# mikelodder7/bls-bn254

Hardware: AMD Instinct MI355X
Metric: BN254 pairings/sec (= BLS verifies/sec) (higher is better)
Workload: dtype int64; 1 GPU; 262144 batched single-sig BLS verifies per GPU (BASELINE configs[1]), unique 32-byte messages, 1024-key pool, 1/64 invalid tuples; key de-duplication + hash-to-G1 + per-key G2 checks and line tables + 2-pair Miller loop + final exp; tuples_per_gpu=262144, tuples_total=262144, key_pool=1024

## Files before the change

bls-bn254_amd/csrc/curve.h:

```cpp
#pragma once
#include "tower.h"

namespace bn {

BN_INL Fp f_add(const Fp& a, const Fp& b) { return fp_add(a, b); }
BN_INL Fp f_sub(const Fp& a, const Fp& b) { return fp_sub(a, b); }
BN_INL Fp f_mul(const Fp& a, const Fp& b) { return fp_mul(a, b); }
BN_INL Fp f_sqr(const Fp& a) { return fp_sqr(a); }
BN_INL Fp f_norm(const Fp& a) { return fp_norm(a); }
BN_INL Fp f_neg(const Fp& a) { return fp_neg(a); }
BN_INL bool f_is_zero(const Fp& a) { return fp_is_zero(a); }
BN_INL Fp f_select(bool c, const Fp& a, const Fp& b) { return fp_select(c, a, b); }
BN_INL Fp f_mul_b3(const Fp& a) { return fp_lc2<9, 0>(a, a); }
template <int K1, int K2> BN_INL Fp f_lc2(const Fp& a, const Fp& b) { return fp_lc2<K1, K2>(a, b); }
template <int K1, int K2, int K3> BN_INL Fp f_lc3(const Fp& a, const Fp& b, const Fp& c) { return fp_lc3<K1, K2, K3>(a, b, c); }
BN_INL void f_set_zero(Fp& a) { a = fp_zero(); }
BN_INL void f_set_one(Fp& a) { a = fp_one(); }

BN_INL Fp2 f_add(const Fp2& a, const Fp2& b) { return fp2_add(a, b); }
BN_INL Fp2 f_sub(const Fp2& a, const Fp2& b) { return fp2_sub(a, b); }
BN_INL Fp2 f_mul(const Fp2& a, const Fp2& b) { return fp2_mul(a, b); }
BN_INL Fp2 f_sqr(const Fp2& a) { return fp2_sqr(a); }
BN_INL Fp2 f_norm(const Fp2& a) { return fp2_norm(a); }
BN_INL Fp2 f_neg(const Fp2& a) { return fp2_neg(a); }
// ... 60 lines not shown
template <class F> BN_FUNC Proj<F> proj_dbl(const Proj<F>& a) {
  BN_CTX;
  F t0 = f_sqr(a.y);
  F z8 = f_lc2<8, 0>(t0, t0);
  F t1 = f_mul(a.y, a.z);
  F t2 = f_mul_b3(f_sqr(a.z));
  F x3 = f_mul(t2, z8);
  F y3 = f_norm(f_add(t0, t2));
  F z3 = f_mul(t1, z8);
  F t0m = f_lc2<1, -3>(t0, t2);
  F yy = f_norm(f_add(x3, f_mul(t0m, y3)));
  F xy = f_mul(a.x, a.y);
  F xx = f_lc2<2, 0>(f_mul(t0m, xy), t0);
  return {xx, yy, z3};
}
template <class F> BN_FUNC Proj<F> jac_dbl(const Proj<F>& p) {
  BN_CTX;
  F A = f_sqr(p.x), B = f_sqr(p.y);
  F C = f_sqr(B);
  F t = f_sqr(f_norm(f_add(p.x, B)));
  F D = f_lc3<2, -2, -2>(t, A, C);
  F E = f_lc2<3, 0>(A, A);
  F x3 = f_lc2<1, -2>(f_sqr(E), D);
  F y3 = f_lc2<1, -8>(f_mul(E, f_norm(f_sub(D, x3))), C);
  F yz = f_mul(p.y, p.z);
  return {x3, y3, f_lc2<2, 0>(yz, yz)};
}
template <class F> BN_FUNC Proj<F> proj_to_jac(const Proj<F>& p) {
  BN_CTX;
  return {f_mul(p.x, p.z), f_mul(p.y, f_sqr(p.z)), p.z};
}
template <class F> BN_FUNC Proj<F> proj_from_jac(const Proj<F>& j) {
  BN_CTX;
  bool inf = f_is_zero(j.z);
  Proj<F> id = proj_identity<F>();
  Proj<F> r = {f_mul(j.x, j.z), j.y, f_mul(f_sqr(j.z), j.z)};
  return {f_select(inf, id.x, r.x), f_select(inf, id.y, r.y), f_select(inf, id.z, r.z)};
}
template <class F> BN_INL Proj<F> proj_neg(const Proj<F>& a) { return {a.x, f_norm(f_neg(a.y)), a.z}; }
template <class F> BN_INL Proj<F> proj_select(bool c, const Proj<F>& a, const Proj<F>& b) {
  return {f_select(c, a.x, b.x), f_select(c, a.y, b.y), f_select(c, a.z, b.z)};
}
template <class F> BN_FUNC Proj<F> proj_mul_u64(const Proj<F>& p, uint64_t k) {
  BN_CTX;
  Proj<F> acc = proj_identity<F>();
  for (int i = 63; i >= 0; --i) {
    acc = proj_dbl(acc);
    if ((k >> i) & 1) acc = proj_add(acc, p);
  }
  return acc;
}
struct ChainOp { int8_t load, sq, mul, store, cstore; };
constexpr int BN_X_CHAIN_LEN = 13, BN_X_CHAIN_SLOTS = 5;
#define BN_X_CHAIN {{-1, 4, 0, 1, 2}, {-1, 1, 0, 3, 4}, {-1, 6, 4, -1, -1}, {-1, 7, 1, -1, -1}, {-1, 2, 3, -1, -1}, {-1, 4, 4, -1, -1}, {-1, 4, 4, -1, -1}, \
                    {-1, 9, 3, -1, -1}, {-1, 4, 3, -1, -1}, {-1, 6, 1, -1, -1}, {-1, 5, 3, -1, -1}, {-1, 5, 2, -1, -1}, {-1, 5, 1, -1, -1}}
template <class F> BN_FUNC Proj<F> proj_mul_bn_x(const Proj<F>& p) {
  BN_CTX;
  const ChainOp prog[BN_X_CHAIN_LEN] = BN_X_CHAIN;
  Proj<F> slot[BN_X_CHAIN_SLOTS];
  slot[0] = p;
  Proj<F> r = p;
  for (int k = 0; k < BN_X_CHAIN_LEN; ++k) {
    const ChainOp op = prog[k];
    if (op.load >= 0) r = slot[op.load];
    if (op.sq >= 2) {
      Proj<F> j = proj_to_jac(r);
      for (int q = 0; q < op.sq; ++q) j = jac_dbl(j);
      r = proj_from_jac(j);
    } else if (op.sq == 1) r = proj_dbl(r);
    if (op.mul >= 0) r = proj_add(r, slot[op.mul]);
    if (op.store >= 0) slot[op.store] = r;
    if (op.cstore >= 0) slot[op.cstore] = proj_neg(r);
  }
  return r;
}
template <class F> BN_FUNC Proj<F> proj_mul_256(const Proj<F>& p, const uint64_t* k) {
  BN_CTX;
  Proj<F> acc = proj_identity<F>();
  for (int i = 255; i >= 0; --i) {
    acc = proj_dbl(acc);
    Proj<F> s = proj_add(acc, p);
    acc = proj_select((k[i >> 6] >> (i & 63)) & 1, s, acc);
  }
  return acc;
}
template <class F> BN_FUNC Proj<F> proj_mul_win4(const Proj<F>& p, const uint64_t* k) {
  BN_CTX;
  Proj<F> tab[16];
  tab[0] = proj_identity<F>();
  tab[1] = p;
  for (int i = 2; i < 16; ++i) tab[i] = proj_add(tab[i - 1], p);
  Proj<F> acc = tab[(int)(k[3] >> 60)];
  for (int w = 62; w >= 0; --w) {
    const int d = (int)((k[w >> 4] >> ((w & 15) * 4)) & 15);
    const Proj<F> t = tab[d];
    acc = proj_dbl(proj_dbl(proj_dbl(proj_dbl(acc))));
    acc = proj_add(acc, t);
  }
  return acc;
}
template <class F> BN_INL bool proj_eq(const Proj<F>& a, const Proj<F>& b) {
  bool ai = f_is_zero(a.z), bi = f_is_zero(b.z);
  bool e = f_is_zero(f_sub(f_mul(a.x, b.z), f_mul(b.x, a.z))) & f_is_zero(f_sub(f_mul(a.y, b.z), f_mul(b.y, a.z)));
  return (ai | bi) ? (ai & bi) : e;
}

BN_INL G1A g1_decode(const uint8_t* b, bool& ok) {
  bool okx, oky;
// ... 102 lines not shown
}
BN_FUNC G1A svdw_g1_finish(const Fp& u_in, const Fp& tv3) {
  BN_CTX;
  Fp u = fp_norm(u_in);
  Fp c2 = fp_const(bnc::SVDW1_C2), c3 = fp_const(bnc::SVDW1_C3), c4 = fp_const(bnc::SVDW1_C4), one = fp_one(), b = fp_const(bnc::THREE);
  Fp u2 = fp_sqr(u);
  Fp tv1 = fp_lc2<4, 0>(u2, u2);
  Fp tv2 = fp_norm(fp_add(one, tv1));
  tv1 = fp_norm(fp_sub(one, tv1));
  Fp tv4 = fp_mul(fp_mul(fp_mul(u, tv1), tv3), c3);
  Fp x1 = fp_norm(fp_sub(c2, tv4));
  Fp gx1 = fp_norm(fp_add(fp_mul(fp_sqr(x1), x1), b));
  Fp x2 = fp_norm(fp_add(c2, tv4));
  Fp gx2 = fp_norm(fp_add(fp_mul(fp_sqr(x2), x2), b));
  Fp x3 = fp_mul(fp_sqr(tv2), tv3);
  x3 = fp_norm(fp_add(fp_mul(fp_sqr(x3), c4), one));
  Fp gx3 = fp_norm(fp_add(fp_mul(fp_sqr(x3), x3), b));
  bool e1 = fp_is_square(gx1), e2 = fp_is_square(gx2), sq;
  G1A r;
  r.x = fp_select(e1, x1, fp_select(e2, x2, x3));
  Fp y = fp_sqrt_cand(fp_select(e1, gx1, fp_select(e2, gx2, gx3)), sq);
  bool flip = fp_sgn0(u) != fp_sgn0(y);
  r.y = fp_select(flip, fp_norm(fp_neg(y)), y);
  r.inf = false;
  return r;
}
BN_FUNC G1A svdw_g1(const Fp& u) { return svdw_g1_finish(u, fp_inv(svdw_g1_den(u))); }
struct SvdwFrac { Fp n, d, y; };
BN_FUNC SvdwFrac svdw_g1_frac(const Fp& u_in) {
  BN_CTX;
  const Fp u = fp_norm(u_in);
  const Fp c2 = fp_const(bnc::SVDW1_C2), c3 = fp_const(bnc::SVDW1_C3), c4 = fp_const(bnc::SVDW1_C4), one = fp_one();
  const Fp u2 = fp_sqr(u);
  Fp tv1 = fp_lc2<4, 0>(u2, u2);
  const Fp tv2 = fp_norm(fp_add(one, tv1));
  tv1 = fp_norm(fp_sub(one, tv1));
  const bool exc = fp_is_zero(tv1) | fp_is_zero(tv2);
  const Fp c3u = fp_mul(c3, u), c2t = fp_mul(c2, tv2);
  const Fp n1 = fp_select(exc, c2, fp_norm(fp_sub(c2t, c3u))), n2 = fp_select(exc, c2, fp_norm(fp_add(c2t, c3u)));
  const Fp d12 = fp_select(exc, one, tv2);
  const Fp t1s = fp_sqr(tv1);
  const Fp d3 = fp_select(exc, one, fp_norm(t1s));
  const Fp n3 = fp_select(exc, one, fp_norm(fp_add(t1s, fp_mul(c4, fp_sqr(tv2)))));
  const Fp v12 = fp_mul(fp_sqr(d12), d12), v3 = fp_mul(fp_sqr(d3), d3);
  const Fp g1n = fp_norm(fp_add(fp_mul(fp_sqr(n1), n1), fp_lc2<3, 0>(v12, v12)));
  const Fp g2n = fp_norm(fp_add(fp_mul(fp_sqr(n2), n2), fp_lc2<3, 0>(v12, v12)));
  const Fp g3n = fp_norm(fp_add(fp_mul(fp_sqr(n3), n3), fp_lc2<3, 0>(v3, v3)));
  const bool e1 = fp_is_square(fp_mul(g1n, d12)), e2 = fp_is_square(fp_mul(g2n, d12));
  SvdwFrac r;
  r.n = fp_select(e1, n1, fp_select(e2, n2, n3));
  r.d = fp_select(e1 | e2, d12, d3);
  const Fp U = fp_select(e1, g1n, fp_select(e2, g2n, g3n)), V = fp_select(e1 | e2, v12, v3);
  const Fp V3 = fp_mul(fp_sqr(V), V);
  const Fp y = fp_mul(fp_mul(U, V), fp_pow(fp_mul(U, V3), BN_EXP(EXP_PM3_4)));
  const bool flip = fp_sgn0(u) != fp_sgn0(y);
  r.y = fp_select(flip, fp_norm(fp_neg(y)), y);
  return r;
}
BN_FUNC G1P hash_to_g1_from_fields_proj(const Fp& u0, const Fp& u1) {
  BN_CTX;
#if defined(__HIP_DEVICE_COMPILE__) && defined(BN_HASH_MAP_LOOP)
  Fp u[2] = {u0, u1};
  G1P q[2];
  _Pragma("unroll 1") for (int k = 0; k < 2; ++k) {
    const SvdwFrac a = svdw_g1_frac(u[k]);
    q[k] = G1P{a.n, fp_mul(a.y, a.d), a.d};
  }
  return proj_add(q[0], q[1]);
#else
  const SvdwFrac a = svdw_g1_frac(u0), b = svdw_g1_frac(u1);
  const G1P q0 = {a.n, fp_mul(a.y, a.d), a.d}, q1 = {b.n, fp_mul(b.y, b.d), b.d};
  return proj_add(q0, q1);
#endif
}
BN_FUNC G1A hash_to_g1_from_fields(const Fp& u0, const Fp& u1) { return g1_to_affine(hash_to_g1_from_fields_proj(u0, u1)); }

BN_FUNC Fp2 fp2_pow(const Fp2& a, Exp256 e) {
  BN_CTX;
  Fp2 base = fp2_norm(a), r = fp2_one();
  for (int i = 255; i >= 0; --i) {
    r = fp2_sqr(r);
    Fp2 m = fp2_mul(r, base);
    r = fp2_select((e.w[i >> 6] >> (i & 63)) & 1, m, r);
  }
  return r;
}
BN_FUNC bool fp2_is_square(const Fp2& a) {
  Fp2 n = fp2_norm(a);
  return fp_is_square(fp_dot2(n.c0, n.c0, n.c1, n.c1));
}
BN_FUNC Fp2 fp2_sqrt(const Fp2& a_in) {
  BN_CTX;
  Fp2 a = fp2_norm(a_in);
  Fp2 a1 = fp2_pow(a, BN_EXP(EXP_PM3_4));
  Fp2 alpha = fp2_mul(fp2_sqr(a1), a);
  Fp2 x0 = fp2_mul(a1, a);
  bool neg_one = fp2_is_zero(fp2_add(alpha, fp2_one()));
  Fp2 alt = {fp_norm(fp_neg(x0.c1)), x0.c0};
  Fp2 b = fp2_pow(fp2_norm(fp2_add(alpha, fp2_one())), BN_EXP(EXP_PM1_2));
  Fp2 r = fp2_mul(b, x0);
  return fp2_select(neg_one, alt, r);
}
BN_FUNC G2A g2_decompress(const uint8_t* in, bool& ok) {
  uint8_t xb[32];
  for (int i = 0; i < 32; ++i) xb[i] = in[i];
  int flag = xb[0] >> 7; xb[0] &= 0x7f;
  bool o0, o1;
// ... 39 lines not shown
```

bls-bn254_amd/csrc/fp29.h:

```cpp
#pragma once
#include <stdint.h>
#include "bn254_consts.h"

#if defined(__HIPCC__)
#include <hip/hip_runtime.h>
#define BN_HD __host__ __device__
#else
#define BN_HD
#endif
#define BN_INL BN_HD inline __attribute__((always_inline))
#ifdef BN_FORCE_INLINE
#define BN_FUNC BN_INL
#else
#define BN_FUNC BN_HD inline
#endif

#define BN_UNROLL _Pragma("unroll")
#if defined(__HIP_DEVICE_COMPILE__)
#define BN_SCHED_BARRIER __builtin_amdgcn_sched_barrier(0)
#else
#define BN_SCHED_BARRIER ((void)0)
#endif

#ifdef BN_CHECK
#include <cmath>
#include <cstdio>
#include <cstdlib>
#endif

namespace bn {

constexpr int NL = 9;
constexpr int RB = 29;
constexpr int32_t MASK = (1 << RB) - 1;

struct Fp {
  int32_t l[NL];
#ifdef BN_CHECK
  double lo = 0, hi = 0;
  double tlo = 0, thi = 0;
  double vb = 0;
#endif
};

#ifdef BN_CHECK
struct CheckStats { double worst_mul = 0, worst_dot = 0, worst_vb = 0; long muls = 0, sqrs = 0, dots = 0, norms = 0, lcs = 0, lc_terms = 0; };
inline CheckStats& check_stats() { static thread_local CheckStats s; return s; }
inline double mag(const Fp& a) { return std::fmax(std::fabs(a.lo), std::fabs(a.hi)); }
inline double tmag(const Fp& a) { return std::fmax(std::fabs(a.tlo), std::fabs(a.thi)); }
struct CtxStack { const char* name[64]; int line[64]; int n = 0; };
inline CtxStack& ctx_stack() { static thread_local CtxStack s; return s; }
struct CtxGuard {
  CtxGuard(const char* f, int l) { CtxStack& s = ctx_stack(); if (s.n < 64) { s.name[s.n] = f; s.line[s.n] = l; } ++s.n; }
  ~CtxGuard() { --ctx_stack().n; }
};
inline void check_fail(const char* what, double v) {
  std::fprintf(stderr, "BN_CHECK violation: %s (%g)\n  context:", what, v);
  CtxStack& s = ctx_stack();
  for (int i = 0; i < s.n && i < 64; ++i) std::fprintf(stderr, " > %s:%d", s.name[i], s.line[i]);
  std::fprintf(stderr, "\n");
  std::abort();
}
#define BN_CTX ::bn::CtxGuard _bn_ctx_guard(__func__, __LINE__)
inline void check_actual(const Fp& a, const char* where) {
  const double L = 536870912.0;
  for (int i = 0; i < NL; ++i) {
    double v = a.l[i] / L, lo = i == NL - 1 ? a.tlo : a.lo, hi = i == NL - 1 ? a.thi : a.hi;
    if (v < lo - 1e-6 || v > hi + 1e-6) { std::fprintf(stderr, "limb %d = %g outside [%g,%g] at %s\n", i, v, lo, hi, where); check_fail("actual limb outside proven interval", v); }
  }
}
inline void set_trk(Fp& r, double lo, double hi, double tlo, double thi, double vb) {
  r.lo = lo; r.hi = hi; r.tlo = tlo; r.thi = thi; r.vb = vb;
  if (vb > check_stats().worst_vb) check_stats().worst_vb = vb;
}
#define BN_TRK(...) __VA_ARGS__
#else
#define BN_TRK(...)
#define BN_CTX
#endif

constexpr double P_OVER_R = 0.0059605;

BN_INL Fp fp_add(const Fp& a, const Fp& b) {
  Fp r;
  BN_UNROLL for (int i = 0; i < NL; ++i) r.l[i] = a.l[i] + b.l[i];
  BN_TRK(set_trk(r, a.lo + b.lo, a.hi + b.hi, a.tlo + b.tlo, a.thi + b.thi, a.vb + b.vb); if (mag(r) >= 3.99 || tmag(r) >= 3.99) check_fail("fp_add limb overflow", mag(r));)
  return r;
}
BN_INL Fp fp_sub(const Fp& a, const Fp& b) {
  Fp r;
  BN_UNROLL for (int i = 0; i < NL; ++i) r.l[i] = a.l[i] - b.l[i];
  BN_TRK(set_trk(r, a.lo - b.hi, a.hi - b.lo, a.tlo - b.thi, a.thi - b.tlo, a.vb + b.vb); if (mag(r) >= 3.99 || tmag(r) >= 3.99) check_fail("fp_sub limb overflow", mag(r));)
  return r;
}
BN_INL Fp fp_neg(const Fp& a) {
  Fp r;
  BN_UNROLL for (int i = 0; i < NL; ++i) r.l[i] = -a.l[i];
  BN_TRK(set_trk(r, -a.hi, -a.lo, -a.thi, -a.tlo, a.vb);)
  return r;
// ... 273 lines not shown
  Fp x;
  words_to_limbs(x.l, w);
  BN_TRK(set_trk(x, 0, 1, 0, 0.04, 6);)
  int32_t c = 0;
  BN_UNROLL for (int i = 0; i < NL; ++i) { int32_t d = x.l[i] - bnc::P[i] + c; c = d >> RB; }
  ok = c < 0;
  return fp_to_mont(x);
}
BN_INL void fp_to_be(uint8_t* b, const Fp& a) {
  Fp c = fp_from_mont(a);
  uint32_t w[8];
  limbs_to_words(w, c.l);
  BN_UNROLL for (int j = 0; j < 8; ++j) store_be32(b + 4 * (7 - j), w[j]);
}
BN_INL Fp fp_from_okm(const uint8_t* okm) {
  uint32_t w[12];
  BN_UNROLL for (int j = 0; j < 12; ++j) w[j] = load_be32(okm + 4 * (11 - j));
  Fp lo, hi;
  BN_UNROLL for (int i = 0; i < NL; ++i) {
    int bit = RB * i, j = bit >> 5, s = bit & 31;
    uint32_t v = w[j] >> s;
    if (s > 32 - RB) v |= w[j + 1] << (32 - s);
    lo.l[i] = (int32_t)(v & (uint32_t)MASK);
  }
  BN_UNROLL for (int i = 0; i < NL; ++i) {
    int bit = RB * (i + NL), j = bit >> 5, s = bit & 31;
    uint32_t v = 0;
    if (j < 12) { v = w[j] >> s; if (s > 32 - RB && j + 1 < 12) v |= w[j + 1] << (32 - s); }
    hi.l[i] = (int32_t)(v & (uint32_t)MASK);
  }
  BN_TRK(set_trk(lo, 0, 1, 0, 1, 170); set_trk(hi, 0, 1, 0, 0, 1e-30);)
  return fp_dot2(lo, fp_const(bnc::R2), hi, fp_const(bnc::R3));
}

struct Exp256 { uint64_t w[4]; };
#define BN_EXP(name) (::bn::Exp256{{bnc::name[0], bnc::name[1], bnc::name[2], bnc::name[3]}})
BN_FUNC Fp fp_pow(const Fp& a, Exp256 e) {
  Fp tab[16];
  tab[0] = fp_one();
  tab[1] = fp_norm(a);
  for (int i = 2; i < 16; ++i) tab[i] = fp_mul(tab[i - 1], tab[1]);
  const uint64_t e0 = e.w[0], e1 = e.w[1], e2 = e.w[2], e3 = e.w[3];
  Fp r = tab[(int)(e3 >> 60)];
  for (int w = 62; w >= 0; --w) {
    uint64_t word = w >= 48 ? e3 : w >= 32 ? e2 : w >= 16 ? e1 : e0;
    int d = (int)((word >> ((w & 15) * 4)) & 15);
    Fp t = tab[d];
    BN_SCHED_BARRIER;
    r = fp_sqr(r); r = fp_sqr(r); r = fp_sqr(r); r = fp_sqr(r);
    r = fp_mul(r, t);
  }
  return r;
}
BN_FUNC Fp fp_inv_pow(const Fp& a) { return fp_pow(a, BN_EXP(EXP_PM2)); }

BN_INL void sg_divsteps29(int32_t& zeta, uint32_t f, uint32_t g, int32_t& u, int32_t& v, int32_t& q, int32_t& r) {
  u = 1; v = 0; q = 0; r = 1;
  BN_UNROLL for (int i = 0; i < RB; ++i) {
    int32_t c1 = zeta >> 31;
    const int32_t c2 = -(int32_t)(g & 1u);
    const uint32_t x = (f ^ (uint32_t)c1) - (uint32_t)c1;
    const int32_t y = (u ^ c1) - c1, z = (v ^ c1) - c1;
    g += x & (uint32_t)c2; q += y & c2; r += z & c2;
    c1 &= c2;
    zeta = (zeta ^ c1) - 1;
    f += g & (uint32_t)c1; u += q & c1; v += r & c1;
    g >>= 1; u *= 2; v *= 2;
  }
}
template <bool MODP>
BN_INL void sg_update(int32_t* a, int32_t* b, int32_t u, int32_t v, int32_t q, int32_t r) {
  int64_t ca = (int64_t)u * a[0] + (int64_t)v * b[0], cb = (int64_t)q * a[0] + (int64_t)r * b[0];
  int32_t ka = 0, kb = 0;
  if (MODP) {
    ka = (int32_t)(((uint32_t)ca * (uint32_t)bnc::PINV) & (uint32_t)MASK); kb = (int32_t)(((uint32_t)cb * (uint32_t)bnc::PINV) & (uint32_t)MASK);
    ca += (int64_t)ka * bnc::P[0]; cb += (int64_t)kb * bnc::P[0];
  }
  ca >>= RB; cb >>= RB;
  BN_UNROLL for (int i = 1; i < NL; ++i) {
    const int32_t ai = a[i], bi = b[i];
    ca += (int64_t)u * ai + (int64_t)v * bi; cb += (int64_t)q * ai + (int64_t)r * bi;
    if (MODP) { ca += (int64_t)ka * bnc::P[i]; cb += (int64_t)kb * bnc::P[i]; }
    a[i - 1] = (int32_t)((uint32_t)ca & (uint32_t)MASK); b[i - 1] = (int32_t)((uint32_t)cb & (uint32_t)MASK);
    ca >>= RB; cb >>= RB;
  }
  a[NL - 1] = (int32_t)ca; b[NL - 1] = (int32_t)cb;
}
constexpr int SG_BATCHES = 21;
BN_FUNC Fp fp_inv_divsteps(const Fp& a, bool& done) {
  const Fp x = fp_from_mont(a);
  int32_t f[NL], g[NL], d[NL], e[NL];
  BN_UNROLL for (int i = 0; i < NL; ++i) { f[i] = bnc::P[i]; g[i] = x.l[i]; d[i] = 0; e[i] = i == 0 ? 1 : 0; }
  int32_t zeta = -1;
  for (int b = 0; b < SG_BATCHES; ++b) {
    int32_t u, v, q, r;
    sg_divsteps29(zeta, (uint32_t)f[0] | ((uint32_t)f[1] << RB), (uint32_t)g[0] | ((uint32_t)g[1] << RB), u, v, q, r);
    sg_update<false>(f, g, u, v, q, r);
    sg_update<true>(d, e, u, v, q, r);
  }
  int32_t gnz = 0;
  BN_UNROLL for (int i = 0; i < NL; ++i) gnz |= g[i];
  done = gnz == 0;
  const bool neg = f[NL - 1] < 0;
  Fp di;
  BN_UNROLL for (int i = 0; i < NL; ++i) di.l[i] = neg ? -d[i] : d[i];
  BN_TRK(set_trk(di, -1, 1, -0.14, 0.14, 22);)
// ... 64 lines not shown
```

bls-bn254_amd/csrc/k_fe_h3.hip:

```cpp
#include "lane_ops.h"
#include "kernels.h"
using namespace bn;


BN_KERNEL k_fe_h3(const int32_t* t, const int32_t* a, const int32_t* c, const int32_t* b2, const int32_t* x0, int32_t* tmp, size_t n, size_t stride,
                  const uint8_t* flags, const uint8_t* sub_ok, uint8_t* bitmap, uint8_t* gt_bytes, int* is_one, int mode) {
  __shared__ int32_t park_lds[108 * 256];
  const uint32_t i = blockIdx.x * blockDim.x + threadIdx.x;
  bool bit = false;
  if (i < n) {
    const uint32_t l4 = i * 4u;
    const Ws src[5] = {{const_cast<int32_t*>(t), stride, l4, true}, {const_cast<int32_t*>(a), stride, l4, true}, {const_cast<int32_t*>(c), stride, l4, true},
                       {const_cast<int32_t*>(b2), stride, l4, true}, {const_cast<int32_t*>(x0), stride, l4, true}};
    const Ws park = {park_lds, 256, threadIdx.x * 4u, false};
    Fp12 r = fe_h3_loop(src, Ws{tmp, stride, l4, true}, &park);
    if (mode == 0) bit = fp12_is_one(r) & (flags[i] == (FLAG_SIG_OK | FLAG_PK_OK)) & (sub_ok[i] != 0);
    else if (mode == 3) *is_one = fp12_is_one(r) ? 1 : 0;
    else if (mode == 4) gt_bytes[i] = fp12_is_one(r) ? 1 : 0;
    else fp12_to_be(gt_bytes + 384 * (size_t)i, r);
  }
  if (mode == 0) write_ballot(bitmap, n, i, bit);
}
```

bls-bn254_amd/csrc/pairing.h:

```cpp
#pragma once
#include "curve.h"

namespace bn {

struct G2J { Fp2 x, y, z; };
struct Line { Fp2 c0, c1, c2; };

BN_FUNC Line doubling_step(G2J& r) {
  BN_CTX;
  Fp2 tmp0 = fp2_sqr(r.x);
  Fp2 tmp1 = fp2_sqr(r.y);
  Fp2 tmp2 = fp2_sqr(tmp1);
  Fp2 s3 = fp2_sqr(fp2_norm(fp2_add(tmp1, r.x)));
  Fp2 tmp3 = f_lc3<2, -2, -2>(s3, tmp0, tmp2);
  Fp2 tmp4 = f_lc2<3, 0>(tmp0, tmp0);
  Fp2 tmp6 = fp2_norm(fp2_add(r.x, tmp4));
  Fp2 tmp5 = fp2_sqr(tmp4);
  Fp2 zsq = fp2_sqr(r.z);
  Fp2 nx = f_lc2<1, -2>(tmp5, tmp3);
  Fp2 nz = fp2_norm(fp2_sub(fp2_sub(fp2_sqr(fp2_norm(fp2_add(r.z, r.y))), tmp1), zsq));
  Fp2 ny = f_lc2<1, -8>(fp2_mul(fp2_sub(tmp3, nx), tmp4), tmp2);
  Line l;
  l.c1 = f_lc2<-2, 0>(fp2_mul(tmp4, zsq), zsq);
  Fp2 s6 = fp2_sub(fp2_sub(fp2_sqr(tmp6), tmp0), tmp5);
// ... 401 lines not shown
  return c;
}
BN_FUNC Fp12 fp12_from_be(const uint8_t* in, bool& ok) {
  BN_CTX;
  ok = true;
  Fp12 a;
  a.c0.c0 = fp2_from_be(in, ok); a.c0.c1 = fp2_from_be(in + 64, ok); a.c0.c2 = fp2_from_be(in + 128, ok);
  a.c1.c0 = fp2_from_be(in + 192, ok); a.c1.c1 = fp2_from_be(in + 256, ok); a.c1.c2 = fp2_from_be(in + 320, ok);
  return a;
}
BN_INL void fp2_store_limbs(int32_t* out, size_t stride, const Fp2& c) {
  Fp c0 = fp_canon(c.c0), c1 = fp_canon(c.c1);
  BN_UNROLL for (int k = 0; k < NL; ++k) { out[(size_t)k * stride] = c0.l[k]; out[(size_t)(9 + k) * stride] = c1.l[k]; }
}
BN_INL void fp2_store_limbs(const Ws& w, const Fp2& c) {
  Fp c0 = fp_canon(c.c0), c1 = fp_canon(c.c1);
  BN_UNROLL for (int k = 0; k < NL; ++k) { ws_store(w, k, c0.l[k]); ws_store(w, 9 + k, c1.l[k]); }
}
BN_FUNC void fp12_store_limbs(const Ws& w, const Fp12& a) {
  BN_CTX;
  fp2_store_limbs(w, a.c0.c0); fp2_store_limbs(ws_at(w, 18), a.c0.c1); fp2_store_limbs(ws_at(w, 36), a.c0.c2);
  fp2_store_limbs(ws_at(w, 54), a.c1.c0); fp2_store_limbs(ws_at(w, 72), a.c1.c1); fp2_store_limbs(ws_at(w, 90), a.c1.c2);
}
BN_INL Fp2 fp2_load_limbs(const Ws& w) {
  Fp2 c;
  BN_UNROLL for (int k = 0; k < NL; ++k) { c.c0.l[k] = ws_load(w, k); c.c1.l[k] = ws_load(w, 9 + k); }
  BN_TRK(set_trk(c.c0, 0, 1, 0, 0.006, 1); set_trk(c.c1, 0, 1, 0, 0.006, 1);)
  return c;
}
BN_FUNC Fp12 fp12_load_limbs(const Ws& w) {
  BN_CTX;
  return {{fp2_load_limbs(w), fp2_load_limbs(ws_at(w, 18)), fp2_load_limbs(ws_at(w, 36))},
          {fp2_load_limbs(ws_at(w, 54)), fp2_load_limbs(ws_at(w, 72)), fp2_load_limbs(ws_at(w, 90))}};
}
BN_FUNC void fp12_store_limbs(int32_t* out, size_t stride, const Fp12& a) {
  BN_CTX;
  fp2_store_limbs(out, stride, a.c0.c0); fp2_store_limbs(out + 18 * stride, stride, a.c0.c1);
  fp2_store_limbs(out + 36 * stride, stride, a.c0.c2); fp2_store_limbs(out + 54 * stride, stride, a.c1.c0);
  fp2_store_limbs(out + 72 * stride, stride, a.c1.c1); fp2_store_limbs(out + 90 * stride, stride, a.c1.c2);
}
BN_INL Fp2 fp2_load_limbs(const int32_t* in, size_t stride) {
  Fp2 c;
  BN_UNROLL for (int k = 0; k < NL; ++k) { c.c0.l[k] = in[(size_t)k * stride]; c.c1.l[k] = in[(size_t)(9 + k) * stride]; }
  BN_TRK(set_trk(c.c0, 0, 1, 0, 0.006, 1); set_trk(c.c1, 0, 1, 0, 0.006, 1);)
  return c;
}
BN_FUNC Fp12 fp12_load_limbs(const int32_t* in, size_t stride) {
  BN_CTX;
  return {{fp2_load_limbs(in, stride), fp2_load_limbs(in + 18 * stride, stride), fp2_load_limbs(in + 36 * stride, stride)},
          {fp2_load_limbs(in + 54 * stride, stride), fp2_load_limbs(in + 72 * stride, stride), fp2_load_limbs(in + 90 * stride, stride)}};
}

struct H3Op { int8_t pre, mul, post; };
BN_FUNC Fp12 fe_h3_loop(const Ws* src, const Ws& tmp, const Ws* park) {
  const H3Op prog[8] = {{1, 4, 1}, {0, 1, 2}, {2, 0, 3}, {3, 2, 0}, {0, 0, 0}, {0, 7, 0}, {0, 6, 0}, {0, 8, 0}};
  Fp12 r = fp12_one();
  for (int k = 0; k < 8; ++k) {
    const H3Op op = prog[k];
    if (op.pre == 1) r = fp12_load_mem(src[3]);
    else if (op.pre == 2) r = fp12_conj(r);
    else if (op.pre == 3) r = fp12_load_mem(tmp);
    const int m = op.mul;
    const Ws b = m == 0 ? src[0] : m == 1 ? src[1] : m == 2 ? src[2] : m == 4 ? src[4] : ws_at(tmp, 108 * (size_t)(m - 5));
    r = fp12_mul_mem(r, b, park);
    if (op.post == 1) { fp12_store_mem(tmp, r); fp12_store_mem(ws_at(tmp, 108), fp12_frob<2>(r)); }
    else if (op.post == 2) fp12_store_mem(ws_at(tmp, 216), fp12_frob<1>(r));
    else if (op.post == 3) fp12_store_mem(ws_at(tmp, 324), fp12_frob<3>(fp12_conj(r)));
    BN_MEM_FENCE;
  }
  return r;
}

BN_FUNC void fe_h1_tail(const Fp12& x0, const Ws& a_out, const Ws& b_out, const Ws* park) {
  Fp12 a = fp12_cyclotomic_sqr(fp12_conj(x0));
  fp12_store_mem(a_out, a);
  BN_MEM_FENCE;
  fp12_store_mem(b_out, fp12_mul_mem(fp12_cyclotomic_sqr(a), a_out, park));
}
BN_FUNC void fe_h2_tail(const Fp12& x0, const Ws& b_in, const Ws& c_out, const Ws& b2_out, const Ws& d2_out, const Ws* park) {
  fp12_store_mem(c_out, fp12_conj(x0));
  BN_MEM_FENCE;
  fp12_store_mem(b2_out, fp12_conj(fp12_mul_mem(x0, b_in, park)));
  BN_MEM_FENCE;
  fp12_store_mem(d2_out, fp12_cyclotomic_sqr(fp12_load_mem(c_out)));
}

BN_INL void line_store_limbs(const Ws& w, const Line& l) { fp2_store_limbs(w, l.c0); fp2_store_limbs(ws_at(w, 18), l.c1); fp2_store_limbs(ws_at(w, 36), l.c2); }
BN_INL Line line_load_limbs(const Ws& w) { return {fp2_load_limbs(w), fp2_load_limbs(ws_at(w, 18)), fp2_load_limbs(ws_at(w, 36))}; }
BN_FUNC void g2_prepare_lines(const G2A& q, const Ws& out) {
  BN_CTX;
  G2J T = {q.x, q.y, fp2_one()};
  Fp2 nqy = fp2_norm(fp2_neg(q.y));
  int ti = 0;
  for (int j = bnc::ATE_NAF_LEN - 2; j >= 0; --j) {
    line_store_limbs(ws_at(out, 54 * (size_t)ti++), doubling_step(T));
    int d = ate_naf_digit(j);
    if (d != 0) line_store_limbs(ws_at(out, 54 * (size_t)ti++), addition_step(T, q.x, d > 0 ? q.y : nqy));
  }
  Fp2 g2 = fp2_const(bnc::GAMMA1[1]), g3 = fp2_const(bnc::GAMMA1[2]);
  Fp2 q1x = fp2_mul(fp2_norm(fp2_conj(q.x)), g2), q1y = fp2_mul(fp2_norm(fp2_conj(q.y)), g3);
  Fp2 q2x = fp2_mul(fp2_norm(fp2_conj(q1x)), g2);
  Fp2 q2y = fp2_norm(fp2_neg(fp2_mul(fp2_norm(fp2_conj(q1y)), g3)));
  line_store_limbs(ws_at(out, 54 * (size_t)ti++), addition_step(T, q1x, q1y));
  line_store_limbs(ws_at(out, 54 * (size_t)ti++), addition_step(T, q2x, q2y));
}
BN_INL void fp_store_limbs_lazy(const Ws& w, const Fp& c) {
  BN_TRK(if (c.lo < -4e-6 || c.hi > 1.0 + 4e-6 || c.tlo < -0.02 || c.thi > 0.02 || c.vb > 1.2) check_fail("pair table entry outside its declared range", c.vb);)
  BN_UNROLL for (int k = 0; k < NL; ++k) ws_store(w, k, c.l[k]);
}
BN_INL Fp fp_load_limbs_lazy(const Ws& w) {
  Fp c;
  BN_UNROLL for (int k = 0; k < NL; ++k) c.l[k] = ws_load(w, k);
  BN_TRK(set_trk(c, -4e-6, 1.0 + 4e-6, -0.02, 0.02, 1.2); check_actual(c, "pair table entry");)
  return c;
}
BN_INL void fp2_store_limbs_lazy(const Ws& w, const Fp2& c) { fp_store_limbs_lazy(w, c.c0); fp_store_limbs_lazy(ws_at(w, 9), c.c1); }
BN_INL Fp2 fp2_load_limbs_lazy(const Ws& w) {
  Fp2 c;
  BN_UNROLL for (int k = 0; k < NL; ++k) { c.c0.l[k] = ws_load(w, k); c.c1.l[k] = ws_load(w, 9 + k); }
  BN_TRK(set_trk(c.c0, -4e-6, 1.0 + 4e-6, -0.02, 0.02, 1.2); set_trk(c.c1, -4e-6, 1.0 + 4e-6, -0.02, 0.02, 1.2);
         check_actual(c.c0, "pair table entry"); check_actual(c.c1, "pair table entry");)
  return c;
}
// ... 218 lines not shown
```

bls-bn254_amd/csrc/sha256.h:

```cpp
#pragma once
#include <stddef.h>
#include <stdint.h>
#include "fp29.h"

namespace bn {

struct Sha256 {
  uint32_t h[8];
  uint32_t w[16];
  uint32_t cur;
  uint32_t fill;
  uint64_t total;
};

BN_INL uint32_t ror32(uint32_t x, int n) { return (x >> n) | (x << (32 - n)); }

#if defined(__HIP_DEVICE_COMPILE__) && !defined(BN_SHA_INLINE)
#define BN_SHA_FUNC BN_HD __attribute__((noinline))
#else
#define BN_SHA_FUNC BN_FUNC
#endif
BN_SHA_FUNC void sha256_compress(uint32_t* h, const uint32_t* blk) {
  const uint32_t K[64] = {
      0x428a2f98, 0x71374491, 0xb5c0fbcf, 0xe9b5dba5, 0x3956c25b, 0x59f111f1, 0x923f82a4, 0xab1c5ed5, 0xd807aa98, 0x12835b01,
      0x243185be, 0x550c7dc3, 0x72be5d74, 0x80deb1fe, 0x9bdc06a7, 0xc19bf174, 0xe49b69c1, 0xefbe4786, 0x0fc19dc6, 0x240ca1cc,
      0x2de92c6f, 0x4a7484aa, 0x5cb0a9dc, 0x76f988da, 0x983e5152, 0xa831c66d, 0xb00327c8, 0xbf597fc7, 0xc6e00bf3, 0xd5a79147,
      0x06ca6351, 0x14292967, 0x27b70a85, 0x2e1b2138, 0x4d2c6dfc, 0x53380d13, 0x650a7354, 0x766a0abb, 0x81c2c92e, 0x92722c85,
      0xa2bfe8a1, 0xa81a664b, 0xc24b8b70, 0xc76c51a3, 0xd192e819, 0xd6990624, 0xf40e3585, 0x106aa070, 0x19a4c116, 0x1e376c08,
      0x2748774c, 0x34b0bcb5, 0x391c0cb3, 0x4ed8aa4a, 0x5b9cca4f, 0x682e6ff3, 0x748f82ee, 0x78a5636f, 0x84c87814, 0x8cc70208,
      0x90befffa, 0xa4506ceb, 0xbef9a3f7, 0xc67178f2};
  uint32_t w[16];
  BN_UNROLL for (int i = 0; i < 16; ++i) w[i] = blk[i];
  uint32_t a = h[0], b = h[1], c = h[2], d = h[3], e = h[4], f = h[5], g = h[6], hh = h[7];
  BN_UNROLL for (int i = 0; i < 64; ++i) {
    if (i >= 16) {
      uint32_t w15 = w[(i - 15) & 15], w2 = w[(i - 2) & 15];
      uint32_t s0 = ror32(w15, 7) ^ ror32(w15, 18) ^ (w15 >> 3);
      uint32_t s1 = ror32(w2, 17) ^ ror32(w2, 19) ^ (w2 >> 10);
      w[i & 15] = w[i & 15] + s0 + w[(i - 7) & 15] + s1;
    }
    uint32_t S1 = ror32(e, 6) ^ ror32(e, 11) ^ ror32(e, 25), ch = (e & f) ^ (~e & g);
    uint32_t t1 = hh + S1 + ch + K[i] + w[i & 15];
    uint32_t S0 = ror32(a, 2) ^ ror32(a, 13) ^ ror32(a, 22), mj = (a & b) ^ (a & c) ^ (b & c);
    uint32_t t2 = S0 + mj;
    hh = g; g = f; f = e; e = d + t1; d = c; c = b; b = a; a = t1 + t2;
  }
  h[0] += a; h[1] += b; h[2] += c; h[3] += d; h[4] += e; h[5] += f; h[6] += g; h[7] += hh;
}
BN_FUNC void sha256_init(Sha256& s) {
  s.h[0] = 0x6a09e667; s.h[1] = 0xbb67ae85; s.h[2] = 0x3c6ef372; s.h[3] = 0xa54ff53a;
  s.h[4] = 0x510e527f; s.h[5] = 0x9b05688c; s.h[6] = 0x1f83d9ab; s.h[7] = 0x5be0cd19;
  for (int i = 0; i < 16; ++i) s.w[i] = 0;
  s.cur = 0; s.fill = 0; s.total = 0;
}
BN_FUNC void sha256_byte(Sha256& s, uint8_t b) {
  s.cur = (s.cur << 8) | b;
  ++s.fill; ++s.total;
  if ((s.fill & 3) == 0) {
    s.w[(s.fill >> 2) - 1] = s.cur;
    s.cur = 0;
    if (s.fill == 64) { sha256_compress(s.h, s.w); s.fill = 0; }
  }
}
BN_FUNC void sha256_update(Sha256& s, const uint8_t* p, size_t n) { for (size_t i = 0; i < n; ++i) sha256_byte(s, p[i]); }
BN_FUNC void sha256_final(Sha256& s, uint8_t* out) {
  uint64_t bits = s.total * 8;
  sha256_byte(s, 0x80);
  while (s.fill != 56) sha256_byte(s, 0);
  for (int i = 0; i < 8; ++i) sha256_byte(s, (uint8_t)(bits >> (8 * (7 - i))));
  for (int i = 0; i < 8; ++i) store_be32(out + 4 * i, s.h[i]);
}

BN_FUNC void expand_message_xmd(uint8_t* out, uint32_t n, const uint8_t* msg, size_t msg_len,
                                     const uint8_t* dst, uint32_t dst_len) {
  uint8_t b0[32], bi[32];
  Sha256 s;
  sha256_init(s);
  for (int i = 0; i < 64; ++i) sha256_byte(s, 0);
  sha256_update(s, msg, msg_len);
  sha256_byte(s, (uint8_t)(n >> 8)); sha256_byte(s, (uint8_t)n); sha256_byte(s, 0);
  sha256_update(s, dst, dst_len); sha256_byte(s, (uint8_t)dst_len);
  sha256_final(s, b0);
  sha256_init(s);
  sha256_update(s, b0, 32); sha256_byte(s, 1);
  sha256_update(s, dst, dst_len); sha256_byte(s, (uint8_t)dst_len);
  sha256_final(s, bi);
  uint32_t ell = (n + 31) / 32, done = 0;
  for (uint32_t i = 1; i <= ell; ++i) {
    for (uint32_t k = 0; k < 32 && done < n; ++k) out[done++] = bi[k];
    if (i == ell) break;
    sha256_init(s);
    for (int k = 0; k < 32; ++k) sha256_byte(s, b0[k] ^ bi[k]);
    sha256_byte(s, (uint8_t)(i + 1));
    sha256_update(s, dst, dst_len); sha256_byte(s, (uint8_t)dst_len);
    sha256_final(s, bi);
  }
}

}
```

Before: 7.988 million verifies/s.

## Shorten BN_X and (p-3)/4 addition chains, precompute SHA zero-pad state, fold final-exp step

Swaps the scalar-by-x addition chain for a different schedule and replaces the generic windowed fp_pow for the SvdW square-root exponent with a dedicated sliding-window addition chain over odd powers. SHA-256 expand_message_xmd now starts from the precomputed state after the 64-byte zero block, which skips one compression per message. The final-exponentiation verdict skips the last multiply and instead compares the partial result with a stored operand, using a conjugate check. These cut field multiplications and hash work, at the cost of hand-derived constants whose correctness depends on the chains being right.

New measurement: 8.079 million verifies/s (median of 6 runs). +1.1%, better.

```diff
diff --git a/bls-bn254_amd/csrc/curve.h b/bls-bn254_amd/csrc/curve.h
--- a/bls-bn254_amd/csrc/curve.h
+++ b/bls-bn254_amd/csrc/curve.h
@@ -136,8 +136,8 @@
 }
 struct ChainOp { int8_t load, sq, mul, store, cstore; };
 constexpr int BN_X_CHAIN_LEN = 13, BN_X_CHAIN_SLOTS = 5;
-#define BN_X_CHAIN {{-1, 4, 0, 1, 2}, {-1, 1, 0, 3, 4}, {-1, 6, 4, -1, -1}, {-1, 7, 1, -1, -1}, {-1, 2, 3, -1, -1}, {-1, 4, 4, -1, -1}, {-1, 4, 4, -1, -1}, \
-                    {-1, 9, 3, -1, -1}, {-1, 4, 3, -1, -1}, {-1, 6, 1, -1, -1}, {-1, 5, 3, -1, -1}, {-1, 5, 2, -1, -1}, {-1, 5, 1, -1, -1}}
+#define BN_X_CHAIN {{-1, 0, -1, -1, 1}, {-1, 7, 0, 2, -1}, {-1, 2, 0, -1, 3}, {-1, 2, 2, 4, -1}, {-1, 4, 2, -1, -1}, {-1, 10, 4, -1, -1}, {-1, 1, 0, -1, -1}, \
+                    {-1, 13, 4, -1, -1}, {-1, 2, 1, -1, -1}, {-1, 5, 0, -1, -1}, {-1, 4, 2, -1, -1}, {-1, 11, 3, -1, -1}, {-1, 1, 3, -1, -1}}
 template <class F> BN_FUNC Proj<F> proj_mul_bn_x(const Proj<F>& p) {
   BN_CTX;
   const ChainOp prog[BN_X_CHAIN_LEN] = BN_X_CHAIN;
@@ -346,7 +346,7 @@
   r.d = fp_select(e1 | e2, d12, d3);
   const Fp U = fp_select(e1, g1n, fp_select(e2, g2n, g3n)), V = fp_select(e1 | e2, v12, v3);
   const Fp V3 = fp_mul(fp_sqr(V), V);
-  const Fp y = fp_mul(fp_mul(U, V), fp_pow(fp_mul(U, V3), BN_EXP(EXP_PM3_4)));
+  const Fp y = fp_mul(fp_mul(U, V), fp_pow_pm3_4(fp_mul(U, V3)));
   const bool flip = fp_sgn0(u) != fp_sgn0(y);
   r.y = fp_select(flip, fp_norm(fp_neg(y)), y);
   return r;
diff --git a/bls-bn254_amd/csrc/fp29.h b/bls-bn254_amd/csrc/fp29.h
--- a/bls-bn254_amd/csrc/fp29.h
+++ b/bls-bn254_amd/csrc/fp29.h
@@ -44,7 +44,7 @@
 };
 
 #ifdef BN_CHECK
-struct CheckStats { double worst_mul = 0, worst_dot = 0, worst_vb = 0; long muls = 0, sqrs = 0, dots = 0, norms = 0, lcs = 0, lc_terms = 0; };
+struct CheckStats { double worst_mul = 0, worst_dot = 0, worst_vb = 0; long muls = 0, sqrs = 0, dots = 0, norms = 0, lcs = 0, lc_terms = 0, sha_blocks = 0; };
 inline CheckStats& check_stats() { static thread_local CheckStats s; return s; }
 inline double mag(const Fp& a) { return std::fmax(std::fabs(a.lo), std::fabs(a.hi)); }
 inline double tmag(const Fp& a) { return std::fmax(std::fabs(a.tlo), std::fabs(a.thi)); }
@@ -424,6 +424,25 @@
   }
   return r;
 }
+struct PowStep { uint8_t sq, idx; };
+constexpr int BN_PM3_4_TAB = 14, BN_PM3_4_FIRST = 1, BN_PM3_4_LEN = 39;
+#define BN_PM3_4_CHAIN {{10, 12}, {8, 9}, {5, 9}, {4, 4}, {4, 3}, {9, 9}, {7, 6}, {10, 2}, {7, 13}, {1, 0}, {7, 2}, {10, 8}, {6, 13}, {5, 6}, {8, 1}, {11, 10}, {1, 0}, {9, 11}, {6, 12}, {5, 7}, {10, 5}, {6, 10}, {7, 8}, {5, 6}, {7, 3}, {6, 3}, {7, 10}, {7, 6}, {6, 7}, {5, 0}, {10, 8}, {1, 0}, {9, 5}, {6, 13}, {8, 7}, {5, 9}, {4, 7}, {4, 2}, {4, 0}}
+BN_FUNC Fp fp_pow_pm3_4(const Fp& a) {
+  const PowStep prog[BN_PM3_4_LEN] = BN_PM3_4_CHAIN;
+  Fp tab[BN_PM3_4_TAB];
+  tab[0] = fp_norm(a);
+  const Fp a2 = fp_sqr(tab[0]);
+  for (int i = 1; i < BN_PM3_4_TAB; ++i) tab[i] = fp_mul(tab[i - 1], a2);
+  Fp r = tab[BN_PM3_4_FIRST];
+  for (int k = 0; k < BN_PM3_4_LEN; ++k) {
+    const PowStep op = prog[k];
+    Fp t = tab[op.idx];
+    BN_SCHED_BARRIER;
+    for (int q = 0; q < op.sq; ++q) r = fp_sqr(r);
+    r = fp_mul(r, t);
+  }
+  return r;
+}
 BN_FUNC Fp fp_inv_pow(const Fp& a) { return fp_pow(a, BN_EXP(EXP_PM2)); }
 
 BN_INL void sg_divsteps29(int32_t& zeta, uint32_t f, uint32_t g, int32_t& u, int32_t& v, int32_t& q, int32_t& r) {
diff --git a/bls-bn254_amd/csrc/k_fe_h3.hip b/bls-bn254_amd/csrc/k_fe_h3.hip
--- a/bls-bn254_amd/csrc/k_fe_h3.hip
+++ b/bls-bn254_amd/csrc/k_fe_h3.hip
@@ -13,11 +13,16 @@
     const Ws src[5] = {{const_cast<int32_t*>(t), stride, l4, true}, {const_cast<int32_t*>(a), stride, l4, true}, {const_cast<int32_t*>(c), stride, l4, true},
                        {const_cast<int32_t*>(b2), stride, l4, true}, {const_cast<int32_t*>(x0), stride, l4, true}};
     const Ws park = {park_lds, 256, threadIdx.x * 4u, false};
-    Fp12 r = fe_h3_loop(src, Ws{tmp, stride, l4, true}, &park);
-    if (mode == 0) bit = fp12_is_one(r) & (flags[i] == (FLAG_SIG_OK | FLAG_PK_OK)) & (sub_ok[i] != 0);
-    else if (mode == 3) *is_one = fp12_is_one(r) ? 1 : 0;
-    else if (mode == 4) gt_bytes[i] = fp12_is_one(r) ? 1 : 0;
-    else fp12_to_be(gt_bytes + 384 * (size_t)i, r);
+    const bool gt_out = mode == 1 || mode == 2;
+    const Ws tw = {tmp, stride, l4, true};
+    Fp12 r = fe_h3_loop(src, tw, &park, gt_out ? 8 : 7);
+    if (gt_out) fp12_to_be(gt_bytes + 384 * (size_t)i, r);
+    else {
+      const bool one = fe_h3_verdict(r, tw);
+      if (mode == 0) bit = one & (flags[i] == (FLAG_SIG_OK | FLAG_PK_OK)) & (sub_ok[i] != 0);
+      else if (mode == 3) *is_one = one ? 1 : 0;
+      else gt_bytes[i] = one ? 1 : 0;
+    }
   }
   if (mode == 0) write_ballot(bitmap, n, i, bit);
 }
diff --git a/bls-bn254_amd/csrc/pairing.h b/bls-bn254_amd/csrc/pairing.h
--- a/bls-bn254_amd/csrc/pairing.h
+++ b/bls-bn254_amd/csrc/pairing.h
@@ -477,10 +477,10 @@
 }
 
 struct H3Op { int8_t pre, mul, post; };
-BN_FUNC Fp12 fe_h3_loop(const Ws* src, const Ws& tmp, const Ws* park) {
+BN_FUNC Fp12 fe_h3_loop(const Ws* src, const Ws& tmp, const Ws* park, int steps = 8) {
   const H3Op prog[8] = {{1, 4, 1}, {0, 1, 2}, {2, 0, 3}, {3, 2, 0}, {0, 0, 0}, {0, 7, 0}, {0, 6, 0}, {0, 8, 0}};
   Fp12 r = fp12_one();
-  for (int k = 0; k < 8; ++k) {
+  for (int k = 0; k < steps; ++k) {
     const H3Op op = prog[k];
     if (op.pre == 1) r = fp12_load_mem(src[3]);
     else if (op.pre == 2) r = fp12_conj(r);
@@ -494,6 +494,19 @@
     BN_MEM_FENCE;
   }
   return r;
+}
+
+BN_FUNC bool fe_h3_verdict(const Fp12& r, const Ws& tmp) {
+  BN_CTX;
+  const Ws b = ws_at(tmp, 324);
+  bool eq = true, zero = true;
+  { const Fp2 x = fp2_load_mem(b); eq &= fp2_eq(r.c0.c0, x); zero &= fp2_is_zero(r.c0.c0); }
+  { const Fp2 x = fp2_load_mem(ws_at(b, 18)); eq &= fp2_eq(r.c0.c1, x); zero &= fp2_is_zero(r.c0.c1); }
+  { const Fp2 x = fp2_load_mem(ws_at(b, 36)); eq &= fp2_eq(r.c0.c2, x); zero &= fp2_is_zero(r.c0.c2); }
+  { const Fp2 x = fp2_load_mem(ws_at(b, 54)); eq &= fp2_is_zero(fp2_add(r.c1.c0, x)); zero &= fp2_is_zero(r.c1.c0); }
+  { const Fp2 x = fp2_load_mem(ws_at(b, 72)); eq &= fp2_is_zero(fp2_add(r.c1.c1, x)); zero &= fp2_is_zero(r.c1.c1); }
+  { const Fp2 x = fp2_load_mem(ws_at(b, 90)); eq &= fp2_is_zero(fp2_add(r.c1.c2, x)); zero &= fp2_is_zero(r.c1.c2); }
+  return eq & !zero;
 }
 
 BN_FUNC void fe_h1_tail(const Fp12& x0, const Ws& a_out, const Ws& b_out, const Ws* park) {
diff --git a/bls-bn254_amd/csrc/sha256.h b/bls-bn254_amd/csrc/sha256.h
--- a/bls-bn254_amd/csrc/sha256.h
+++ b/bls-bn254_amd/csrc/sha256.h
@@ -29,6 +29,7 @@
       0xa2bfe8a1, 0xa81a664b, 0xc24b8b70, 0xc76c51a3, 0xd192e819, 0xd6990624, 0xf40e3585, 0x106aa070, 0x19a4c116, 0x1e376c08,
       0x2748774c, 0x34b0bcb5, 0x391c0cb3, 0x4ed8aa4a, 0x5b9cca4f, 0x682e6ff3, 0x748f82ee, 0x78a5636f, 0x84c87814, 0x8cc70208,
       0x90befffa, 0xa4506ceb, 0xbef9a3f7, 0xc67178f2};
+  BN_TRK(++check_stats().sha_blocks;)
   uint32_t w[16];
   BN_UNROLL for (int i = 0; i < 16; ++i) w[i] = blk[i];
   uint32_t a = h[0], b = h[1], c = h[2], d = h[3], e = h[4], f = h[5], g = h[6], hh = h[7];
@@ -53,6 +54,12 @@
   for (int i = 0; i < 16; ++i) s.w[i] = 0;
   s.cur = 0; s.fill = 0; s.total = 0;
 }
+BN_FUNC void sha256_init_zpad(Sha256& s) {
+  s.h[0] = 0xda5698be; s.h[1] = 0x17b9b469; s.h[2] = 0x62335799; s.h[3] = 0x779fbeca;
+  s.h[4] = 0x8ce5d491; s.h[5] = 0xc0d26243; s.h[6] = 0xbafef9ea; s.h[7] = 0x1837a9d8;
+  for (int i = 0; i < 16; ++i) s.w[i] = 0;
+  s.cur = 0; s.fill = 0; s.total = 64;
+}
 BN_FUNC void sha256_byte(Sha256& s, uint8_t b) {
   s.cur = (s.cur << 8) | b;
   ++s.fill; ++s.total;
@@ -75,8 +82,7 @@
                                      const uint8_t* dst, uint32_t dst_len) {
   uint8_t b0[32], bi[32];
   Sha256 s;
-  sha256_init(s);
-  for (int i = 0; i < 64; ++i) sha256_byte(s, 0);
+  sha256_init_zpad(s);
   sha256_update(s, msg, msg_len);
   sha256_byte(s, (uint8_t)(n >> 8)); sha256_byte(s, (uint8_t)n); sha256_byte(s, 0);
   sha256_update(s, dst, dst_len); sha256_byte(s, (uint8_t)dst_len);
```
